# MasterXiong/Hyper-VLA

Measured on AMD Instinct MI355X. Metric: actions_per_sec, higher is better.
Workload: dtype f16; 1 GPU; BASELINE configs[1]: hypernet weight-gen once (untimed) + full sample_actions step (u8 224x224 -> DINOv2-base E=768 in the loop -> generated vit_t 4L/64d policy -> [4,7] action chunk); 1 action = 1 sample-step; batch_per_gpu=256, global_batch=256, encoder=DINOv2-base (reference parity, E=768), parallelism=episode-dp1 (no collectives), policy_operands=split-bf16 (bf16x3), launch=eager (114 launches per step, counted by the library), streams=1, ensemble=not in the step

## Files before the change

hyper-vla_amd/csrc/encoder.hip:

```cpp
#include <cstring>
#include <type_traits>

#include "common.h"
#include "kernels.h"
#include "plan.h"

namespace hvla {

template <typename Op>
__global__ void im2col_kernel(const uint8_t* __restrict__ img, typename Op::elem* __restrict__ out, int B,
                              int image, int patch, int grid, int Kp, float* __restrict__ x, const float* __restrict__ pos, int S, int E) {
  for (size_t i = (size_t)blockIdx.x * blockDim.x + threadIdx.x; i < (size_t)B * E; i += (size_t)gridDim.x * blockDim.x)
    x[(i / E) * S * E + (i % E)] = pos[i % E];
  const int Kp1 = Kp / 2, chunks = Kp1 / 8;
  const size_t total = (size_t)B * grid * grid * chunks;
  const int kreal = patch * patch * 3;
  for (size_t i = (size_t)blockIdx.x * blockDim.x + threadIdx.x; i < total; i += (size_t)gridDim.x * blockDim.x) {
    const int ch = (int)(i % chunks);
    const size_t m = i / chunks;
    const int px = (int)(m % grid), py = (int)((m / grid) % grid);
    const size_t b = m / ((size_t)grid * grid);
    typename Op::x8 v;
    const int rowb = 3 * patch;
    const int k0 = ch * 8;
    int dy = k0 / rowb, rb = k0 - dy * rowb;
    const uint8_t* src = img + ((b * image + (size_t)(py * patch + dy)) * image + (size_t)px * patch) * 3;
#pragma unroll
    for (int j = 0; j < 8; ++j) {
      float f = 0.f;
      if (k0 + j < kreal) f = (float)src[rb] - 128.f;
      v[j] = (typename Op::elem)f;
      if (++rb == rowb) rb = 0, src += (size_t)image * 3;
    }
    *reinterpret_cast<typename Op::x8*>(out + m * Kp + ch * 8) = v;
    *reinterpret_cast<typename Op::x8*>(out + m * Kp + Kp1 + ch * 8) = v;
  }
}

struct GemmArgs {
  const void* A;
  const void* W;
  int M, N, K;
  const float* bias;
  const float* aux;
  void* out;
  int P, S;
  int qcols;
  float qscale;
  const float* corr = nullptr;
  const void* abar2 = nullptr;
  const void* dW2 = nullptr;
  float* corr2 = nullptr;
  int M2 = 0;
  int row0 = 0, row_step = 1;
  int hsplit = 1 << 30;
  int tile_row0 = 0, tile_stride = 256, nbm = 0;
  void* colmean = nullptr;
  void* ln_out = nullptr;
  const float* ln_scale = nullptr;
  const float* ln_bias = nullptr;
  void* ln_abar = nullptr;
  uint32_t* ln_cnt = nullptr;
  float* ln_part = nullptr;
  uint32_t ln_target = 0;
  uint32_t ln_tag = 0;
  uint32_t ln_spin = 0;
  uint32_t out_bytes = 0;
  uint32_t part_bytes = 0;
  int lnx_G = 0, lnx_rows_aligned = 0, lnx_rounds_div = 0, lnx_rows_xcd = 0, lnx_rcp = 0;
  const float* ln_partial = nullptr;
};

__device__ __forceinline__ int wperm(int rho) { return (rho & ~63) + 4 * (rho & 15) + ((rho >> 4) & 3); }
__device__ __forceinline__ f32x4 corr_value(f32x4 acc, float b) {
  return f32x4{fmaf(acc[0], 1.f / 4096.f, b), fmaf(acc[1], 1.f / 4096.f, b), fmaf(acc[2], 1.f / 4096.f, b), fmaf(acc[3], 1.f / 4096.f, b)};
}

template <typename Op, int EPI, int MT, bool FULL, bool ROWBIAS, bool CS = false, bool WT = false, bool NT = false>
__device__ __forceinline__ void gemm_epilogue_rows_impl(const f32x4 (&acc)[4][MT], const GemmArgs& g, int m_base, int n_base,
                                                        int fr, int fq, const f32x4* pre_b4, const f32x4* pre_l4,
                                                        typename Op::x4* cs = nullptr,
                                                        const __attribute__((address_space(3))) float* lds_corr = nullptr,
                                                        int lds_img0 = -1) {
  using T = typename Op::elem;
  const int n = n_base + 4 * fr;
  f32x4 b4 = f32x4{0.f, 0.f, 0.f, 0.f};
  if constexpr (!ROWBIAS) b4 = pre_b4 ? *pre_b4 : *reinterpret_cast<const f32x4*>(g.bias + n);
  f32x4 l4 = f32x4{1.f, 1.f, 1.f, 1.f};
  if constexpr (EPI == EPI_RES) l4 = pre_l4 ? *pre_l4 : *reinterpret_cast<const f32x4*>(g.aux + n);
  const float q = EPI == EPI_PATCH ? g.qscale : ((EPI == EPI_QKV && n_base < g.qcols) ? g.qscale : 1.f);
  __amdgpu_buffer_rsrc_t wt_rsrc;
  if constexpr (WT) wt_rsrc = __builtin_amdgcn_make_buffer_rsrc(g.out, 0, (int)g.out_bytes, 0x00020000);
  auto store_f32x4 = [&](uint32_t elem_off, f32x4 v) {
    if constexpr (WT) __builtin_amdgcn_raw_buffer_store_b128(__builtin_bit_cast(u32x4, v), wt_rsrc, (int)(elem_off * 4u), 0, 16);
    else *reinterpret_cast<f32x4*>(reinterpret_cast<float*>(g.out) + elem_off) = v;
  };
  __amdgpu_buffer_rsrc_t nt_rsrc;
  uint32_t nt_vo = 0;
  if constexpr (NT && FULL && (EPI == EPI_QKV || EPI == EPI_GELU)) {
    nt_rsrc = __builtin_amdgcn_make_buffer_rsrc(g.out, 0, -1, 0x00020000);
    nt_vo = ((uint32_t)(g.row0 + (m_base + 4 * fq) * g.row_step) * (uint32_t)g.N + (uint32_t)n) * (uint32_t)sizeof(T);
  }
  constexpr int RB = MT < 2 ? 1 : (EPI == EPI_RES && MT >= 4 ? 4 : 2);
#pragma unroll
  for (int mp = 0; mp < MT; mp += RB) {
    f32x4 xin[RB][4], brow[RB][4];
    uint32_t off[RB][4];
    bool ok[RB][4];
#pragma unroll
    for (int u = 0; u < RB; ++u)
#pragma unroll
      for (int r = 0; r < 4; ++r) {
        const int m = m_base + (mp + u) * 16 + 4 * fq + r;
        ok[u][r] = FULL || m < g.M;
        const int grow = g.row0 + m * g.row_step;
        off[u][r] = (uint32_t)grow * (uint32_t)g.N + (uint32_t)n;
        if constexpr (EPI == EPI_PATCH) {
          const int prow = 1 + (m % g.P);
// ... 34 lines not shown
        if constexpr (EPI == EPI_GELU) {
          const f32x2 g0 = gelu_erf2(f32x2{t[c][0], t[c][1]}), g1 = gelu_erf2(f32x2{t[c][2], t[c][3]});
          t[c] = f32x4{g0[0], g0[1], g1[0], g1[1]};
        }
      }
#pragma unroll
      for (int r = 0; r < 4; ++r) {
        if (!ok[u][r]) continue;
        if constexpr (EPI == EPI_QKV || EPI == EPI_GELU) {
          typename Op::x4 o;
#pragma unroll
          for (int c = 0; c < 4; ++c) o[c] = (T)t[c][r];
          if constexpr (CS) *cs += o;
          if constexpr (NT && FULL) {
            int rowb = g.row_step * g.N * (int)sizeof(T);
            asm volatile("" : "+s"(rowb));
            __builtin_amdgcn_raw_buffer_store_b64(__builtin_bit_cast(u32x2, o), nt_rsrc, (int)nt_vo, ((mp + u) * 16 + r) * rowb, 2);
          } else if constexpr (NT) __builtin_nontemporal_store(o, reinterpret_cast<typename Op::x4*>(reinterpret_cast<T*>(g.out) + off[u][r]));
          else *reinterpret_cast<typename Op::x4*>(reinterpret_cast<T*>(g.out) + off[u][r]) = o;
        } else if constexpr (EPI == EPI_RES) {
          f32x4 x = xin[u][r];
#pragma unroll
          for (int c = 0; c < 4; ++c) x[c] = fmaf(t[c][r], l4[c], x[c]);
          store_f32x4(off[u][r], x);
        } else if constexpr (EPI == EPI_CORR) {
          *reinterpret_cast<f32x4*>(reinterpret_cast<float*>(g.out) + off[u][r]) = f32x4{t[0][r], t[1][r], t[2][r], t[3][r]};
        } else {
          f32x4 x = xin[u][r];
#pragma unroll
          for (int c = 0; c < 4; ++c) x[c] += t[c][r];
          store_f32x4(off[u][r], x);
        }
      }
    }
  }
}

template <typename Op, int EPI, int MT>
__device__ __forceinline__ void gemm_epilogue_rows(const f32x4 (&acc)[4][MT], const GemmArgs& g, int m_base, int n_base,
                                                   int fr, int fq) {
  const bool full = m_base + 16 * MT <= g.M;
  if constexpr (EPI == EPI_PATCH || EPI == EPI_CORR) {
    if (full) gemm_epilogue_rows_impl<Op, EPI, MT, true, false>(acc, g, m_base, n_base, fr, fq, nullptr, nullptr);
    else gemm_epilogue_rows_impl<Op, EPI, MT, false, false>(acc, g, m_base, n_base, fr, fq, nullptr, nullptr);
  } else {
    if (g.corr) {
      if (full) gemm_epilogue_rows_impl<Op, EPI, MT, true, true>(acc, g, m_base, n_base, fr, fq, nullptr, nullptr);
      else gemm_epilogue_rows_impl<Op, EPI, MT, false, true>(acc, g, m_base, n_base, fr, fq, nullptr, nullptr);
    } else {
      if (full) gemm_epilogue_rows_impl<Op, EPI, MT, true, false>(acc, g, m_base, n_base, fr, fq, nullptr, nullptr);
      else gemm_epilogue_rows_impl<Op, EPI, MT, false, false>(acc, g, m_base, n_base, fr, fq, nullptr, nullptr);
    }
  }
}


template <typename Op, int EPI>
__global__ __launch_bounds__(256, 2) void gemm_kernel(GemmArgs g) {
  using T = typename Op::elem;
  using X8 = typename Op::x8;
  extern __shared__ __attribute__((aligned(16))) char smem[];
  T* As = reinterpret_cast<T*>(smem);
  T* Ws = As + 2 * GBM * GLD;
  const int tid = threadIdx.x, wave = tid >> 6, lane = tid & 63;
  const int wm = wave >> 1, wn = wave & 1;
  const int nbm = (g.M + GBM - 1) / GBM, nbn = g.N / GBN;
  const int bid = xcd_run(blockIdx.x, nbm * nbn);
  const int bm = bid % nbm, bn = bid / nbm;
  const int m0 = bm * GBM, n0 = bn * GBN;
  const T* A = reinterpret_cast<const T*>(g.A);
  const T* W = reinterpret_cast<const T*>(g.W);

  const int lrow = tid >> 3, lch = tid & 7;
  const T* ap[4];
  const T* wp[4];
#pragma unroll
  for (int i = 0; i < 4; ++i) {
    int m = m0 + lrow + 32 * i;
    m = m < g.M ? m : g.M - 1;
    ap[i] = A + (size_t)(g.row0 + m * g.row_step) * g.K + lch * 8;
    wp[i] = W + (size_t)(n0 + wperm(lrow + 32 * i)) * g.K + lch * 8;
  }
  X8 ra[4], rw[4];
  auto gload = [&](int kt) {
#pragma unroll
    for (int i = 0; i < 4; ++i) {
      ra[i] = *reinterpret_cast<const X8*>(ap[i] + kt * GBK);
      rw[i] = *reinterpret_cast<const X8*>(wp[i] + kt * GBK);
    }
  };
  auto sstore = [&](int buf) {
#pragma unroll
    for (int i = 0; i < 4; ++i) {
      *reinterpret_cast<X8*>(As + (buf * GBM + lrow + 32 * i) * GLD + lch * 8) = ra[i];
      *reinterpret_cast<X8*>(Ws + (buf * GBN + lrow + 32 * i) * GLD + lch * 8) = rw[i];
    }
  };

  f32x4 acc[4][4];
#pragma unroll
  for (int i = 0; i < 4; ++i)
#pragma unroll
    for (int j = 0; j < 4; ++j) acc[i][j] = f32x4{0.f, 0.f, 0.f, 0.f};

  const int KT = g.K / GBK;
  gload(0);
  sstore(0);
  __syncthreads();
  const int fr = lane & 15, fq = lane >> 4;
  for (int kt = 0; kt < KT; ++kt) {
    const int buf = kt & 1;
    if (kt + 1 < KT) gload(kt + 1);
    const T* as = As + (buf * GBM + wm * 64 + fr) * GLD + fq * 8;
    const T* ws = Ws + (buf * GBN + wn * 64 + fr) * GLD + fq * 8;
#pragma unroll
    for (int kk = 0; kk < 2; ++kk) {
      X8 fa[4], fw[4];
#pragma unroll
      for (int t = 0; t < 4; ++t) {
        fa[t] = *reinterpret_cast<const X8*>(as + t * 16 * GLD + kk * 32);
        fw[t] = *reinterpret_cast<const X8*>(ws + t * 16 * GLD + kk * 32);
      }
#pragma unroll
      for (int nt = 0; nt < 4; ++nt)
#pragma unroll
        for (int mt = 0; mt < 4; ++mt) acc[nt][mt] = Op::mma16(fa[mt], fw[nt], acc[nt][mt]);
    }
    if (kt + 1 < KT) sstore(buf ^ 1);
    __syncthreads();
  }

  gemm_epilogue_rows<Op, EPI, 4>(acc, g, m0 + wm * 64, n0 + wn * 64, fr, fq);
}

template <typename Op, int EPI, int NS = SNS>
__device__ __forceinline__ void gemm64_body(const GemmArgs& g, int bm, int bn) {
  using T = typename Op::elem;
  using X8 = typename Op::x8;
  extern __shared__ __attribute__((aligned(16))) char smem[];
  const int tid = threadIdx.x, lane = tid & 63;
  const int wave = __builtin_amdgcn_readfirstlane(tid >> 6);
  const int m0 = bm * SBM, n0 = bn * SBN;
  const T* A = reinterpret_cast<const T*>(g.A);
  const T* W = reinterpret_cast<const T*>(g.W);
  const int sch = ((lane & 7) ^ (lane >> 3)) * 8;
  uint32_t aoff[2], woff[2];
#pragma unroll
  for (int j = 0; j < 2; ++j) {
    const int rl = 32 * j + 8 * wave + (lane >> 3);
    int m = m0 + rl;
    m = m < g.M ? m : g.M - 1;
    aoff[j] = (uint32_t)(g.row0 + m * g.row_step) * (uint32_t)g.K + sch;
    woff[j] = (uint32_t)(n0 + wperm(rl)) * (uint32_t)g.K + sch;
  }
  const int KT = g.K / 64;
  auto issue = [&](int kt) {
    char* base = smem + (kt % NS) * 16384 + wave * 1024;
#pragma unroll
    for (int j = 0; j < 2; ++j) {
      __builtin_amdgcn_global_load_lds((const __attribute__((address_space(1))) void*)(A + aoff[j] + kt * 64),
                                       (__attribute__((address_space(3))) void*)(base + j * 4096), 16, 0, 0);
      __builtin_amdgcn_global_load_lds((const __attribute__((address_space(1))) void*)(W + woff[j] + kt * 64),
                                       (__attribute__((address_space(3))) void*)(base + 8192 + j * 4096), 16, 0, 0);
    }
  };
  f32x4 acc[4][1];
#pragma unroll
  for (int i = 0; i < 4; ++i) acc[i][0] = f32x4{0.f, 0.f, 0.f, 0.f};
  const int fr = lane & 15, fq = lane >> 4;
  const int sw0 = (fq ^ (fr & 7)) << 4, sw1 = ((fq + 4) ^ (fr & 7)) << 4;
  const int a_off = (wave * 16 + fr) * 128, w_off = 8192 + fr * 128;
#pragma unroll
  for (int s = 0; s < NS - 1; ++s)
    if (s < KT) issue(s);
  for (int kt = 0; kt < KT; ++kt) {
    const int issued = kt + NS - 1 < KT ? kt + NS - 1 : KT;
    switch (issued - kt - 1) {
      case 0: asm volatile("s_waitcnt vmcnt(0)" ::: "memory"); break;
      case 1: asm volatile("s_waitcnt vmcnt(4)" ::: "memory"); break;
      case 2: asm volatile("s_waitcnt vmcnt(8)" ::: "memory"); break;
      case 3: asm volatile("s_waitcnt vmcnt(12)" ::: "memory"); break;
      default: asm volatile("s_waitcnt vmcnt(16)" ::: "memory"); break;
    }
    __builtin_amdgcn_sched_barrier(0);
    __builtin_amdgcn_s_barrier();
    asm volatile("" ::: "memory");
    __builtin_amdgcn_sched_barrier(0);
    const char* lb = smem + (kt % NS) * 16384;
    X8 fa[2], fw[4][2];
    fa[0] = *reinterpret_cast<const X8*>(lb + a_off + sw0);
    fa[1] = *reinterpret_cast<const X8*>(lb + a_off + sw1);
#pragma unroll
    for (int nt = 0; nt < 4; ++nt) {
      fw[nt][0] = *reinterpret_cast<const X8*>(lb + w_off + nt * 2048 + sw0);
      fw[nt][1] = *reinterpret_cast<const X8*>(lb + w_off + nt * 2048 + sw1);
    }
    __builtin_amdgcn_sched_barrier(0);
    if (kt + NS - 1 < KT) issue(kt + NS - 1);
    asm volatile("s_waitcnt lgkmcnt(0)" ::: "memory");
    __builtin_amdgcn_sched_barrier(0);
#pragma unroll
    for (int kk = 0; kk < 2; ++kk)
#pragma unroll
      for (int nt = 0; nt < 4; ++nt) acc[nt][0] = Op::mma16(fa[kk], fw[nt][kk], acc[nt][0]);
  }
  gemm_epilogue_rows<Op, EPI, 1>(acc, g, m0 + wave * 16, n0, fr, fq);
}

template <typename Op, int EPI, int NS = SNS>
__global__ __launch_bounds__(256) void gemm64_kernel(GemmArgs g) {
  const int nbm1 = (g.M + SBM - 1) / SBM, nbm2 = (g.M2 + SBM - 1) / SBM, rt_all = nbm1 + nbm2;
  const int t = xcd_run(blockIdx.x, gridDim.x);
  const int bn = t / rt_all, bm = t - bn * rt_all;
  if (bm < nbm1) {
    gemm64_body<Op, EPI, NS>(g, bm, bn);
  } else {
    GemmArgs c = g;
    c.A = g.abar2; c.W = g.dW2; c.out = g.corr2; c.M = g.M2; c.row0 = 0; c.row_step = 1; c.corr = nullptr;
    gemm64_body<Op, EPI_CORR, NS>(c, bm - nbm1, bn);
  }
}

__device__ __forceinline__ f32x4 ln_half_sum(const f32x4* p, int n4) { return (p[0] + p[n4]) + (p[2 * n4] + p[3 * n4]); }
template <typename Op, int EPI, bool FOLD = false>
__global__ __launch_bounds__(256) void gemm64c_kernel(GemmArgs g) {
  constexpr int SST = FOLD ? SSTF : SSTC, PCS = FOLD ? 6 : 7;
  using T = typename Op::elem;
  using X8 = typename Op::x8;
  extern __shared__ __attribute__((aligned(16))) char smem[];
  const int tid = threadIdx.x, lane = tid & 63;
  const int wave = __builtin_amdgcn_readfirstlane(tid >> 6);
  const int nbm = (g.M + SBM - 1) / SBM;
  const int tix = xcd_run(blockIdx.x, gridDim.x), bm = tix % nbm, bn = tix / nbm;
  const int m0 = bm * SBM, n0 = bn * SBN;
  const T* A = reinterpret_cast<const T*>(g.A);
  const T* W = reinterpret_cast<const T*>(g.W);
  const T* dW = reinterpret_cast<const T*>(g.dW2);
  const T* AB = reinterpret_cast<const T*>(g.abar2);
  const int img0 = (g.row0 + m0 * g.row_step) / g.S;
  const int sch = ((lane & 7) ^ (lane >> 3)) * 8;
  uint32_t aoff[2], woff[2], boff;
#pragma unroll
  for (int j = 0; j < 2; ++j) {
    const int rl = 32 * j + 8 * wave + (lane >> 3);
    int m = m0 + rl;
    m = m < g.M ? m : g.M - 1;
    aoff[j] = (uint32_t)(g.row0 + m * g.row_step) * (uint32_t)g.K + sch;
    woff[j] = (uint32_t)(n0 + wperm(rl)) * (uint32_t)g.K + sch;
  }
  {
    int mr = img0 * 2 + 8 * wave + (lane >> 3);
    mr = mr < g.M2 ? mr : g.M2 - 1;
    boff = (uint32_t)mr * (uint32_t)g.K + sch;
  }
  const int KT = g.K / 64;
  const uint32_t lds0 = (uint32_t)(uintptr_t)(__attribute__((address_space(3))) char*)smem;
  auto dma = [&](const T* sb, uint32_t elem_off, uint32_t dst) {
    const uint32_t vo = elem_off * (uint32_t)sizeof(T);
    uint32_t keep;
    asm volatile("s_mov_b32 %0, m0\n\ts_mov_b32 m0, %3\n\ts_nop 0\n\tglobal_load_lds_dwordx4 %1, %2\n\ts_mov_b32 m0, %0"
                 : "=&s"(keep) : "v"(vo), "s"(sb), "s"(dst));
  };
  auto issue_at = [&](int kt, int slot) {
    const uint32_t base = lds0 + (uint32_t)((slot % SNSC) * SST + wave * 1024);
#pragma unroll
    for (int j = 0; j < 2; ++j) {
      dma(A, aoff[j] + kt * 64, base + j * 4096);
      dma(W, woff[j] + kt * 64, base + 8192 + j * 4096);
      dma(dW, woff[j] + kt * 64, base + 16384 + j * 4096);
    }
    if constexpr (!FOLD) dma(AB, boff + kt * 64, base + 24576);
  };
  f32x4 acc[4][1], acc2 = f32x4{0.f, 0.f, 0.f, 0.f};
#pragma unroll
  for (int i = 0; i < 4; ++i) acc[i][0] = f32x4{0.f, 0.f, 0.f, 0.f};
  const int fr = lane & 15, fq = lane >> 4;
  const int sw0 = (fq ^ (fr & 7)) << 4, sw1 = ((fq + 4) ^ (fr & 7)) << 4;
  const int a_off = (wave * 16 + fr) * 128, w_off = 8192 + fr * 128;
  const int d_off = 16384 + (wave * 16 + fr) * 128, b_off = 24576 + fr * 128;
#pragma unroll
  for (int s = 0; s < SNSC - 1; ++s) issue_at(s < KT ? s : KT - 1, s);
  char* mtab = smem + SNSC * SST;
  if constexpr (FOLD) {
    int mlast = m0 + SBM - 1;
    mlast = mlast < g.M ? mlast : g.M - 1;
    const int nr = 2 * ((g.row0 + mlast * g.row_step) / g.S - img0 + 1);
    const int n4 = g.K / 4;
    for (int it = tid; it < nr * n4; it += 256) {
      const int r = it / n4, c4 = it - r * n4, bh = img0 * 2 + r;
      const f32x4 t = ln_half_sum(reinterpret_cast<const f32x4*>(g.ln_partial + (size_t)bh * 4 * g.K) + c4, n4);
      const float inv = 1.f / (float)(g.P / 2);
      typename Op::x4 o;
#pragma unroll
      for (int j = 0; j < 4; ++j) o[j] = (T)(t[j] * inv);
      const int k = 4 * c4;
      *reinterpret_cast<typename Op::x4*>(mtab + (k >> 6) * 2048 + r * 128 + ((((k & 63) >> 3) ^ (r & 7)) << 4) + (k & 7) * 2) = o;
    }
  }
  struct Frags {
    X8 fa[2], fw[4][2], fb[2], fd[2];
  };
  auto read_frags = [&](int t, Frags& f) {
    const char* lb = smem + (t % SNSC) * SST;
    f.fa[0] = *reinterpret_cast<const X8*>(lb + a_off + sw0);
    f.fa[1] = *reinterpret_cast<const X8*>(lb + a_off + sw1);
#pragma unroll
    for (int nt = 0; nt < 4; ++nt) {
      f.fw[nt][0] = *reinterpret_cast<const X8*>(lb + w_off + nt * 2048 + sw0);
      f.fw[nt][1] = *reinterpret_cast<const X8*>(lb + w_off + nt * 2048 + sw1);
// ... 338 lines not shown
  const int bh = blockIdx.x, n4 = E / 4;
  if ((int)threadIdx.x >= n4) return;
  const f32x4 t = ln_half_sum(reinterpret_cast<const f32x4*>(partial + (size_t)bh * 4 * E) + threadIdx.x, n4);
  const float inv = 1.f / (float)(P / 2);
  typename Op::x4 o;
#pragma unroll
  for (int j = 0; j < 4; ++j) o[j] = (typename Op::elem)(t[j] * inv);
  reinterpret_cast<typename Op::x4*>(abar + (size_t)bh * E)[threadIdx.x] = o;
}
constexpr int PRO_DMA = 12, PRO_DMA_KT0 = 8;
template <int EPI> struct EpiVmem { static constexpr int min_ops = (EPI == EPI_RES || EPI == EPI_PATCH) ? 64 : 32; };

#ifdef HVLA_BENCH_HOOKS
__device__ unsigned long long g_lnx_dbg[8][256];
#endif
constexpr int LNX_STAT = 98304, LNX_MR = LNX_STAT + 8192, LNX_CTRL = LNX_MR + 2048;
typedef __attribute__((address_space(3))) char lds_char;
template <typename Op, int EPI, bool PERSIST, bool LNX = false, bool NTOUT = false>
__global__ __launch_bounds__(512) void gemm256p_kernel(GemmArgs g) {
  static_assert(!NTOUT || EPI != EPI_PATCH, "NTOUT: non-temporal stores of the 16-bit outputs (QKV, GELU) / loads of the residual rows (RES)");
  using T = typename Op::elem;
  using X8 = typename Op::x8;
  static_assert(!LNX || EPI == EPI_RES || EPI == EPI_PATCH, "the fused LayerNorm follows a GEMM that writes the residual stream");
  extern __shared__ __attribute__((aligned(16))) char smem[];
  const int tid = threadIdx.x, lane = tid & 63;
  const int wave = __builtin_amdgcn_readfirstlane(tid >> 6);
  const int wm = wave >> 2, wn = wave & 3;
  const int nbm = g.nbm, nbn = (g.N + HBN_ - 1) / HBN_;
  const int ntiles = nbm * nbn;
  const int GN = nbn % 4 == 0 ? 4 : (nbn % 3 == 0 ? 3 : (nbn % 2 == 0 ? 2 : 1));
  auto tile_origin = [&](int v, int& tm, int& n0) {
    const int q = ntiles / 8, r = ntiles % 8, xcd = v % 8;
    const int bid = (xcd < r ? xcd * (q + 1) : r * (q + 1) + (xcd - r) * q) + v / 8;
    constexpr int CH = 8;
    const int per_chunk = CH * nbn;
    const int chunk = bid / per_chunk, rc = bid % per_chunk;
    const int rows = (nbm - chunk * CH) < CH ? (nbm - chunk * CH) : CH;
    const int sc = rc / (rows * GN), r2 = rc % (rows * GN);
    tm = chunk * CH + r2 / GN;
    n0 = (sc * GN + r2 % GN) * HBN_;
  };
  bool later = false;
  int rnd = 0;
  int pend_img = -1;
  uint32_t pend_mark = 0;
  auto tile_origin_x = [&](int& tm, int& n0, bool& lat) {
    typedef const __attribute__((address_space(4))) GemmArgs* karg_ptr;
    karg_ptr ga = (karg_ptr)__builtin_amdgcn_kernarg_segment_ptr();
    asm volatile("" : "+s"(ga));
    const int xcd = (int)blockIdx.x & 7, w = (int)blockIdx.x >> 3;
    const int G = ga->lnx_G, rcp = ga->lnx_rcp, wq = (w * rcp) >> 16, rq = (rnd * rcp) >> 16;
    int row, col;
    if (wq < G) {
      row = rnd * G + wq; col = w - wq * nbn; lat = false;
    } else {
      row = ga->lnx_rows_aligned + (w - G * nbn) * ga->lnx_rounds_div + rq; col = rnd - rq * nbn; lat = col != nbn - 1;
    }
    tm = xcd * ga->lnx_rows_xcd + row;
    n0 = col * HBN_;
    ++rnd;
  };
  int vb = blockIdx.x, tm, n0;
  if constexpr (LNX && PERSIST) tile_origin_x(tm, n0, later);
  else tile_origin(vb, tm, n0);
  int m0 = g.tile_row0 + tm * g.tile_stride;
  const T* A = reinterpret_cast<const T*>(g.A);
  const T* W = reinterpret_cast<const T*>(g.W);
  const int srow = wave * 8 + (lane >> 3);
  const int sch = ((lane & 7) ^ (lane >> 3)) * 8;
  const uint32_t lane_a = ((uint32_t)srow * (uint32_t)g.K + sch) * (uint32_t)sizeof(T);
  const uint32_t lane_w = ((uint32_t)(wperm(srow)) * (uint32_t)g.K + sch) * (uint32_t)sizeof(T);
  const uint32_t lds0 = (uint32_t)(uintptr_t)(__attribute__((address_space(3))) char*)smem;
  const T* abase = A + (size_t)m0 * g.K;
  const T* wbase = W + (size_t)n0 * g.K;
  int wn0 = n0;
  const int KT = g.K / 64;
  auto stage = [&](auto hc, int kt) {
    constexpr int h = decltype(hc)::value;
    const int buf = kt & 1;
#pragma unroll
    for (int u = 0; u < 2; ++u) {
      const int j = 2 * (h & 1) + u;
      const int jw = (h < 2 || wn0 + 64 * j < g.N) ? j : 0;
      const T* sb = (h < 2 ? abase : wbase) + ((size_t)jw * 64 * g.K + kt * 64);
      const uint32_t dst = lds0 + (uint32_t)(buf * 65536 + wave * 1024 + (h >> 1) * 32768 + j * 8192);
      const uint32_t vo = h < 2 ? lane_a : lane_w;
      uint32_t keep;
      asm volatile("s_mov_b32 %0, m0\n\ts_mov_b32 m0, %3\n\ts_nop 0\n\tglobal_load_lds_dwordx4 %1, %2\n\ts_mov_b32 m0, %0"
                   : "=&s"(keep) : "v"(vo), "s"(sb), "s"(dst));
    }
  };
  f32x4 acc[4][8];
  const int fr = lane & 15, fq = lane >> 4;
  const int sw0 = ((fq) ^ (fr & 7)) << 4, sw1 = ((fq + 4) ^ (fr & 7)) << 4;
  const int a_off = (wm * 128 + fr) * 128, w_off = 32768 + (wn * 64 + fr) * 128;
  X8 fa0[8], fa1[8], fw0[4], fw1[4];
  auto rd_a = [&](X8 (&f)[8], const char* lb, int ah) {
#pragma unroll
    for (int t = 0; t < 4; ++t) {
      f[2 * t] = *reinterpret_cast<const X8*>(lb + a_off + (4 * ah + t) * 2048 + sw0);
      f[2 * t + 1] = *reinterpret_cast<const X8*>(lb + a_off + (4 * ah + t) * 2048 + sw1);
    }
  };
  auto rd_w = [&](X8 (&f)[4], const char* lb, int wh) {
#pragma unroll
    for (int t = 0; t < 2; ++t) {
      f[2 * t] = *reinterpret_cast<const X8*>(lb + w_off + (2 * wh + t) * 2048 + sw0);
      f[2 * t + 1] = *reinterpret_cast<const X8*>(lb + w_off + (2 * wh + t) * 2048 + sw1);
    }
  };
  auto quad = [&](const X8 (&fa)[8], const X8 (&fw)[4], auto ahc, auto whc) {
    constexpr int ah = decltype(ahc)::value, wh = decltype(whc)::value;
#pragma unroll
    for (int kk = 0; kk < 2; ++kk)
#pragma unroll
      for (int mt = 0; mt < 4; ++mt)
#pragma unroll
        for (int nt = 0; nt < 2; ++nt)
          acc[2 * wh + nt][4 * ah + mt] = Op::mma16(fa[2 * mt + kk], fw[2 * nt + kk], acc[2 * wh + nt][4 * ah + mt]);
  };
  using H0 = std::integral_constant<int, 0>;
  using H1 = std::integral_constant<int, 1>;
  using H2 = std::integral_constant<int, 2>;
  using H3 = std::integral_constant<int, 3>;
#define HVLA_BAR() do { __builtin_amdgcn_sched_barrier(0); __builtin_amdgcn_s_barrier(); __builtin_amdgcn_sched_barrier(0); } while (0)
  stage(H0{}, 0); stage(H1{}, 0); stage(H2{}, 0); stage(H3{}, 0);
  if (KT > 1) {
    stage(H0{}, 1); stage(H1{}, 1);
    asm volatile("s_waitcnt vmcnt(4)" ::: "memory");
  } else {
    asm volatile("s_waitcnt vmcnt(0)" ::: "memory");
  }
  auto ktile = [&](int kt, auto s1c, auto s2c) {
    constexpr bool S1 = decltype(s1c)::value, S2 = decltype(s2c)::value;
    const char* lb = smem + (kt & 1) * 65536;
    rd_w(fw0, lb, 0);
    rd_a(fa0, lb, 0);
    if constexpr (S1) stage(H2{}, kt + 1);
    HVLA_BAR();
    asm volatile("s_waitcnt lgkmcnt(0)" ::: "memory");
    quad(fa0, fw0, H0{}, H0{});
    HVLA_BAR();
    rd_w(fw1, lb, 1);
    rd_a(fa1, lb, 1);
    if constexpr (S1) stage(H3{}, kt + 1);
    asm volatile("s_waitcnt lgkmcnt(0)" ::: "memory");
    HVLA_BAR();
    quad(fa0, fw1, H0{}, H1{});
    HVLA_BAR();
    if constexpr (S2) stage(H0{}, kt + 2);
    HVLA_BAR();
    quad(fa1, fw1, H1{}, H1{});
    HVLA_BAR();
    if constexpr (S2) stage(H1{}, kt + 2);
    if constexpr (S2) asm volatile("s_waitcnt vmcnt(4)" ::: "memory");
    else if constexpr (S1) asm volatile("s_waitcnt vmcnt(0)" ::: "memory");
    HVLA_BAR();
    quad(fa1, fw0, H1{}, H0{});
    HVLA_BAR();
  };
  using Yes = std::integral_constant<bool, true>;
  using No = std::integral_constant<bool, false>;
  while (true) {
#pragma unroll
    for (int i = 0; i < 4; ++i)
#pragma unroll
      for (int j = 0; j < 8; ++j) acc[i][j] = f32x4{0.f, 0.f, 0.f, 0.f};
// ... 969 lines not shown
  for (size_t i = (size_t)blockIdx.x * blockDim.x + threadIdx.x; i < n8; i += (size_t)gridDim.x * blockDim.x) {
    const x8 v = reinterpret_cast<const x8*>(p)[i];
#pragma unroll
    for (int j = 0; j < 8; ++j) {
      const float f = fabsf((float)v[j]);
      if (!(f <= 3.0e38f)) ++bad;
      else mx = fmaxf(mx, f);
    }
  }
#pragma unroll
  for (int o = 32; o >= 1; o >>= 1) {
    mx = fmaxf(mx, __shfl_xor(mx, o, 64));
    bad += __shfl_xor(bad, o, 64);
  }
  if ((threadIdx.x & 63) == 0) {
    atomicMax(slot, __float_as_uint(mx));
    if (bad) atomicAdd(slot + 1, bad);
  }
}

template <typename Op>
struct EncKernels {
  typedef void (*Gemm)(GemmArgs);
  typedef decltype(&attention_kernel<Op, false>) Attn;
  static const Gemm* gemm() {
    static const Gemm t[NUM_GEMM_KERNELS] = {
#define HVLA_X(id, ...) __VA_ARGS__,
        HVLA_GEMM_KERNELS(HVLA_X)
#undef HVLA_X
    };
    return t;
  }
  static const Attn* attn() {
    static const Attn t[NUM_ATTN_KERNELS] = {attention_kernel<Op, false>, attention_kernel<Op, false, 8>, attention_kernel<Op, true>};
    return t;
  }
  static auto ln_group() { return layernorm_group_kernel<Op>; }
  static hipError_t raise_lds_limit() {
    auto raise = [](auto kern) { return hipFuncSetAttribute(reinterpret_cast<const void*>(kern), hipFuncAttributeMaxDynamicSharedMemorySize, (int)LDS_LIMIT); };
    hipError_t e = raise(ln_group());
    for (int k = 0; k < NUM_GEMM_KERNELS && e == hipSuccess; ++k) e = raise(gemm()[k]);
    for (int k = 0; k < NUM_ATTN_KERNELS && e == hipSuccess; ++k) e = raise(attn()[k]);
    return e;
  }
};

namespace {
struct DeviceInfo {
  bool attr[2] = {false, false};
  int ncu = 0;
};
DeviceInfo g_dev[64];
}
template <typename Op>
static hipError_t device_setup(int& ncu) {
  constexpr int opi = std::is_same<Op, OpBF16>::value ? 1 : 0;
  int dev = 0;
  hipError_t e = hipGetDevice(&dev);
  if (e != hipSuccess) return e;
  if (dev < 0 || dev >= 64) return hipErrorInvalidDevice;
  DeviceInfo& di = g_dev[dev];
  if (!di.attr[opi]) {
    if ((e = EncKernels<Op>::raise_lds_limit()) != hipSuccess) return e;
    di.attr[opi] = true;
  }
  if (!di.ncu && (hipDeviceGetAttribute(&di.ncu, hipDeviceAttributeMultiprocessorCount, dev) != hipSuccess || di.ncu <= 0)) di.ncu = 256;
  ncu = di.ncu;
  return hipSuccess;
}
static dim3 grid_of(const Launch& l) { return dim3(l.grid, l.grid_y); }

#define HVLA_LAUNCH(...) do { ++pf.nlaunch; hipLaunchKernelGGL(__VA_ARGS__); } while (0)
template <typename Op>
static hipError_t run_encoder(const Geom& g, const EncWeights& w, const EncWorkspace& ws, const uint8_t* images,
                              float* tokens, int B, hipStream_t st, Profiler* prof, bool keep_cls, uint32_t* audit) {
  Profiler none;
  Profiler& pf = prof ? *prof : none;
  using T = typename Op::elem;
  using Kern = EncKernels<Op>;
  const int P = g.P(), S = g.S(), E = g.E, F = g.enc_mlp, H = g.enc_heads, M = B * S;
  const bool comp = w.layer[0].dqkv != nullptr && ws.corr && ws.abar;
  EncSizes z{B, P, S, E, F, H, g.patch, g.enc_layers, 0, sizeof(T), comp, ws.ln_cnt != nullptr && ws.ln_part != nullptr, ws.amap != nullptr};
  const CallPlan call = plan_call(z);
  if (!call.ok) return hipErrorInvalidValue;
  hipError_t e = device_setup<Op>(z.ncu);
  if (e != hipSuccess) return e;
  const int hsplit = 1 + P / 2;
  bool ln_fused = false;
  uint32_t ln_launch = 0;
  const float* ln_partial = nullptr;
  auto gemm = [&](int epi, GemmArgs a, const void* dW, int cat, const float* ln_s = nullptr, const float* ln_b = nullptr, void* colmean = nullptr) -> bool {
    const GemmPlan p = plan_gemm(z, epi, a.N, a.K, cat, ln_s != nullptr, ln_partial != nullptr);
    if (p.small) {
      GemmArgs c = a;
      if (p.aligned) {
        c.M = B; c.row0 = 0; c.row_step = S;
        if (comp) { c.abar2 = ws.abar; c.dW2 = dW; c.corr2 = ws.corr; c.M2 = 2 * B; }
      } else {
        c = GemmArgs{ws.abar, dW, 2 * B, a.N, a.K, a.bias, nullptr, ws.corr, P, S, 0, 1.f};
      }
      pf.begin(p.small.cat, st);
      HVLA_LAUNCH(Kern::gemm()[p.small.kernel], grid_of(p.small), dim3(p.small.block), p.small.lds, st, c);
      pf.end(p.small.cat, st);
    }
    if (p.aligned) {
      a.nbm = p.nbm; a.tile_row0 = p.tile_row0; a.tile_stride = p.tile_stride; a.colmean = colmean;
      if (epi != EPI_PATCH) a.corr = comp ? ws.corr : nullptr;
    } else if (p.fused_bias) {
      a.abar2 = ws.abar; a.dW2 = dW; a.M2 = 2 * B;
      if (p.fold) { a.ln_partial = ln_partial; ln_partial = nullptr; }
    } else if (p.small) {
      a.corr = ws.corr;
    }
    if (p.ln_fused) {
      a.hsplit = hsplit;
      a.ln_out = ws.h; a.ln_scale = ln_s; a.ln_bias = ln_b; a.ln_abar = comp ? ws.abar : nullptr; a.ln_cnt = ws.ln_cnt; a.ln_part = ws.ln_part;
      a.out_bytes = (uint32_t)((size_t)M * E * 4);
      a.part_bytes = (uint32_t)((size_t)B * p.nbn * 256 * 16);
      a.ln_tag = ++ln_launch;
      a.ln_target = ln_launch * (uint32_t)p.nbn;
      a.ln_spin = ws.ln_spin;
      a.lnx_G = p.lnx_G; a.lnx_rows_aligned = p.lnx_rows_aligned; a.lnx_rounds_div = p.lnx_rounds_div; a.lnx_rows_xcd = p.lnx_rows_xcd; a.lnx_rcp = p.lnx_rcp;
    }
    ln_fused = p.ln_fused;
    const int bracket = epi == EPI_PATCH ? -1 : p.main.cat;
    pf.begin(bracket, st);
    HVLA_LAUNCH(Kern::gemm()[p.main.kernel], grid_of(p.main), dim3(p.main.block), p.main.lds, st, a);
    pf.end(bracket, st);
    return p.aligned;
  };
  auto layer_gemm = [&](const void* A, const void* Wt, int N, int K, const float* bias, const float* aux, void* out, int qcols) {
    GemmArgs a{A, Wt, M, N, K, bias, aux, out, P, S, qcols, qcols ? 0.125f * 1.4426950408889634f : 1.f / 256.f};
    a.hsplit = hsplit;
    return a;
  };
  auto layernorm = [&](const float* sc, const float* bi, int Nnext, void* scratch, int scratch_cols) {
    const NormPlan n = plan_norm(z, Nnext, scratch_cols);
    float* partial = n.partial ? reinterpret_cast<float*>(scratch) : nullptr;
    pf.begin(n.group.cat, st);
    HVLA_LAUNCH(Kern::ln_group(), grid_of(n.group), dim3(n.group.block), n.group.lds, st, ws.x, reinterpret_cast<T*>(ws.h), sc, bi, partial, S, P, E);
    if (n.fold) ln_partial = partial;
    else if (n.mean) HVLA_LAUNCH((layernorm_mean_kernel<Op>), grid_of(n.mean), dim3(n.mean.block), 0, st, partial, reinterpret_cast<T*>(ws.abar), P, E);
    pf.end(n.group.cat, st);
  };
  auto audit_of = [&](const void* buf, size_t n, int site) {
    if (!audit) return;
    HVLA_LAUNCH((absmax_kernel<T>), dim3(1024), dim3(256), 0, st, reinterpret_cast<const T*>(buf), n / 8, audit + 2 * site);
  };
  if (call.cnt_bytes) {
    if ((e = hipMemsetAsync(ws.ln_cnt, 0, call.cnt_bytes, st)) != hipSuccess) return e;
    if ((e = hipMemsetAsync(ws.ln_part, 0, call.part_bytes, st)) != hipSuccess) return e;
    pf.nlaunch += 2;
  }
  pf.begin(call.im2col.cat, st);
  HVLA_LAUNCH(im2col_kernel<Op>, grid_of(call.im2col), dim3(call.im2col.block), 0, st, images, reinterpret_cast<T*>(ws.g), B,
              g.image_size, g.patch, g.grid(), call.Kp, ws.x, w.pos, S, E);
  gemm(EPI_PATCH, GemmArgs{ws.g, w.w_patch, B * P, E, call.Kp, w.b_patch, w.pos, ws.x, P, S, 0, 1.f / 256.f}, nullptr, call.im2col.cat,
       g.enc_layers > 0 ? w.layer[0].ln1_s : nullptr, g.enc_layers > 0 ? w.layer[0].ln1_b : nullptr);
  pf.end(call.im2col.cat, st);
#ifdef HVLA_BENCH_HOOKS
  int products = 0;
#define HVLA_STOP_HERE() do { if (ws.stop_after > 0 && ++products == ws.stop_after) return hipGetLastError(); } while (0)
#else
#define HVLA_STOP_HERE() do { } while (0)
#endif
  for (int l = 0; l < g.enc_layers; ++l) {
    const EncLayerW& L = w.layer[l];
// ... 101 lines not shown
```

hyper-vla_amd/csrc/plan.h:

```cpp
#pragma once
#include <stddef.h>
#include <stdint.h>

#ifdef __HIPCC__
#define HVLA_HD __host__ __device__ __forceinline__
#else
#define HVLA_HD inline
#endif

namespace hvla {

HVLA_HD int xcd_run(int bid, int nwg) {
  const int q = nwg / 8, r = nwg % 8, xcd = bid % 8;
  return (xcd < r ? xcd * (q + 1) : r * (q + 1) + (xcd - r) * q) + bid / 8;
}

HVLA_HD bool big_output(size_t rows, size_t cols, size_t elem_bytes) { return rows * cols * elem_bytes >= ((size_t)96 << 20); }

HVLA_HD bool nt16_addressable(size_t rows, size_t cols, size_t elem_bytes) { return rows * cols * elem_bytes < ((size_t)1 << 32); }

enum { EPI_PATCH = 0, EPI_QKV = 1, EPI_GELU = 2, EPI_RES = 3, EPI_CORR = 4 };
constexpr int GBM = 128, GBN = 128, GBK = 64, GLD = 72;
constexpr int SBM = 64, SBN = 64, SNS = 6, SST = 16384;
constexpr int SNSC = 5, SSTC = 28672;
// ... 91 lines not shown
    const int Wx = z.ncu / 8, R = p.nbm * p.nbn / z.ncu;
    p.lnx_G = Wx / p.nbn; p.lnx_rows_aligned = R * p.lnx_G; p.lnx_rounds_div = R / p.nbn; p.lnx_rows_xcd = p.nbm / 8;
    p.lnx_rcp = (65536 + p.nbn - 1) / p.nbn;
  }
}
inline GemmPlan plan_gemm(const EncSizes& z, int epi, int N, int K, int cat, bool ln_follows, bool ln_partial) {
  GemmPlan p;
  const int B = z.B, ncu = z.ncu, M = epi == EPI_PATCH ? B * z.P : z.M();
  const bool fits32 = (size_t)M * K < (1ull << 31) && (epi == EPI_PATCH || (size_t)N * K < (1ull << 31));
  p.main.block = 256;
  p.main.cat = cat;
  p.nbn = ceil_div(N, HBN_);
  p.aligned = N % SBN == 0 && N >= HBN_ && M > G64_MAXM && fits32 &&
              (epi == EPI_PATCH ? M % HBM_ == 0 : z.P == HBM_ && K >= 128 && K % 64 == 0);
  if (p.aligned) {
    p.main.block = 512;
    p.main.lds = P256_LDS;
    if (epi == EPI_PATCH) {
      p.nbm = M / HBM_; p.tile_row0 = 0; p.tile_stride = HBM_;
      if (z.P == HBM_ && can_fuse_ln(z) && ln_follows) { plan_lnx(z, p, G256LN_PATCH); return p; }
    } else {
      int nblocks = ceil_div(B, SBM) * (N / SBN);
      if (z.comp) nblocks += ceil_div(2 * B, SBM) * (N / SBN);
      const bool two_per_cu = nblocks > ncu;
      p.small = Launch{two_per_cu ? G64S4_QKV - EPI_QKV + epi : G64_PATCH + epi, (unsigned)nblocks, 1, 256, (size_t)(two_per_cu ? 4 : SNS) * SST, CAT_COMP};
      p.nbm = B; p.tile_row0 = 1; p.tile_stride = z.S;
      if (epi == EPI_RES && ln_follows && can_fuse_ln(z)) {
        plan_lnx(z, p, big_output(M, N, sizeof(float)) ? G256LNNT_RES : G256LN_RES);
        return p;
      }
      if (big_output(M, N, epi == EPI_RES ? sizeof(float) : z.elem) && (epi == EPI_RES || nt16_addressable(M, N, z.elem))) {
        const bool persist = (B * p.nbn) % ncu == 0;
        p.main.kernel = G256NT_QKV + 2 * (epi - EPI_QKV) + persist;
        p.main.grid = persist ? ncu : B * p.nbn;
        return p;
      }
    }
    const bool persist = (p.nbm * p.nbn) % ncu == 0;
    p.main.kernel = G256_PATCH + 2 * epi + persist;
    p.main.grid = persist ? ncu : p.nbm * p.nbn;
    return p;
  }
  if (epi != EPI_PATCH && small_fused(z, N, K)) {
    const int nb64 = ceil_div(M, SBM) * (N / SBN);
    p.fused_bias = true;
    if (epi != EPI_RES && ln_partial) {
      p.fold = true;
      p.main.kernel = G64CF_QKV - EPI_QKV + epi; p.main.grid = nb64; p.main.lds = gemm64c_fold_lds(K);
    } else if (epi == EPI_RES && 2 * nb64 <= ncu) {
      p.main.kernel = G64C32; p.main.grid = 2 * nb64; p.main.lds = (size_t)SNS32 * SST32;
    } else {
      p.main.kernel = G64C_QKV - EPI_QKV + epi; p.main.grid = nb64; p.main.lds = (size_t)SNSC * SSTC;
    }
    return p;
  }
  if (epi != EPI_PATCH && z.comp)
    p.small = Launch{G64_CORR, (unsigned)(ceil_div(2 * B, SBM) * (N / SBN)), 1, 256, (size_t)SNS * SST, CAT_COMP};
  if (M <= G64_MAXM && fits32 && N % SBN == 0 && (epi == EPI_PATCH || K % 64 == 0)) {
    p.main.kernel = G64_PATCH + epi; p.main.grid = ceil_div(M, SBM) * (N / SBN); p.main.lds = (size_t)SNS * SST;
  } else {
    p.main.kernel = G128_PATCH + epi; p.main.grid = ceil_div(M, GBM) * (N / GBN); p.main.lds = (size_t)2 * (GBM + GBN) * GLD * z.elem;
  }
  return p;
}

struct NormPlan {
  Launch group, mean;
  bool partial = false, fold = false;
};
inline NormPlan plan_norm(const EncSizes& z, int Nnext, int scratch_cols) {
  NormPlan n;
  n.group = Launch{LN_GROUP, LNG, (unsigned)z.B, LNW * 64, (size_t)(z.P / 8) * z.E * sizeof(float), 1};
  n.partial = z.comp && (size_t)LNG * z.E * sizeof(float) <= (size_t)z.S * scratch_cols * z.elem;
  n.fold = n.partial && small_fused(z, Nnext, z.E) && gemm64c_fold_lds(z.E) <= LDS_LIMIT && ceil_div(z.M(), SBM) * (Nnext / SBN) <= z.ncu;
  if (n.partial && !n.fold) n.mean = Launch{LN_MEAN, 2u * z.B, 1, 256, 0, 1};
  return n;
}

inline Launch plan_attention(int B, int S, int H, size_t elem, bool amap) {
  const int KT = (S + 31) / 32;
  return Launch{amap ? ATT_MAP : KT == 9 ? ATT_U : ATT, (unsigned)(B * H), 1, (unsigned)(KT - 1) * 64, attention_lds(KT, elem, amap), 3};
}

struct CallPlan {
  bool ok = false;
  int Kp = 0;
  size_t cnt_bytes = 0, part_bytes = 0;
  Launch im2col, attention, colmean, final_norm;
};
inline CallPlan plan_call(const EncSizes& z) {
  CallPlan c;
  const int M = z.M();
  c.ok = (size_t)M * (size_t)(z.F > 3 * z.E ? z.F : 3 * z.E) < (1ull << 32);
  if (!c.ok) return c;
  c.Kp = 2 * ((z.patch * z.patch * 3 + 63) / 64 * 64);
  if (can_fuse_ln(z) && z.P == HBM_ && M > G64_MAXM) {
    c.cnt_bytes = (size_t)((z.B * 4 + 15) / 16 * 16);
    c.part_bytes = (size_t)z.B * ceil_div(z.E, HBN_) * 256 * 16;
  }
  const size_t chunks = ((size_t)z.B * z.P * (c.Kp / 16) + 255) / 256;
  c.im2col = Launch{IM2COL, (unsigned)(chunks > 8192 ? 8192 : chunks), 1, 256, 0, 0};
  c.attention = plan_attention(z.B, z.S, z.H, z.elem, z.amap);
  if (z.comp) c.colmean = Launch{COLMEAN, (unsigned)ceil_div(z.F, 256), (unsigned)z.B, 256, 0, -1};
  c.final_norm = Launch{LN_FINAL, (unsigned)ceil_div(M, 4), 1, 256, 0, 1};
  return c;
}

}
```

Measured before the change: 19080 actions/s.

## Stage image strips in LDS for im2col and drop duplicated patch operand half

im2col now loads each full patch-row strip of the image into shared memory with aligned nontemporal 16-byte loads, then gathers patch elements from LDS instead of doing byte-wise global reads. It also writes only the first half of the split-bf16 patch operand. The patch GEMMs remap the A k-tile index for the second half back onto the first, so the duplicate copy is never materialised. This cuts global write traffic and uncoalesced reads in the patch-embedding stage, at the cost of a new LDS staging path with fallback conditions and a Kp%128 requirement.

Result: no change. 19110 actions/s, median of 6 (+0.2%).

```diff
diff --git a/hyper-vla_amd/csrc/encoder.hip b/hyper-vla_amd/csrc/encoder.hip
--- a/hyper-vla_amd/csrc/encoder.hip
+++ b/hyper-vla_amd/csrc/encoder.hip
@@ -7,21 +7,70 @@
 
 namespace hvla {
 
+constexpr int IM2COL_STRIP = 12288;
 template <typename Op>
 __global__ void im2col_kernel(const uint8_t* __restrict__ img, typename Op::elem* __restrict__ out, int B,
                               int image, int patch, int grid, int Kp, float* __restrict__ x, const float* __restrict__ pos, int S, int E) {
   for (size_t i = (size_t)blockIdx.x * blockDim.x + threadIdx.x; i < (size_t)B * E; i += (size_t)gridDim.x * blockDim.x)
     x[(i / E) * S * E + (i % E)] = pos[i % E];
   const int Kp1 = Kp / 2, chunks = Kp1 / 8;
+  const int kreal = patch * patch * 3;
+  const int rowb = 3 * patch, imgrow = 3 * image;
+  __shared__ __attribute__((aligned(16))) uint8_t strip[IM2COL_STRIP];
+  const int strip_bytes = patch * imgrow;
+  if (imgrow % 16 == 0 && (reinterpret_cast<uintptr_t>(img) & 15) == 0 && strip_bytes <= IM2COL_STRIP &&
+      strip_bytes <= 48 * (int)blockDim.x && chunks <= (int)blockDim.x && grid * patch <= image) {
+    const int tid = threadIdx.x, nthr = blockDim.x;
+    const int rpp = nthr / chunks;
+    const int pxo = tid / chunks, ch = tid - pxo * chunks;
+    int off[8];
+    uint32_t live = 0;
+    {
+      const int k0 = ch * 8;
+      int dy = k0 / rowb, rb = k0 - dy * rowb;
+#pragma unroll
+      for (int j = 0; j < 8; ++j) {
+        const bool real = k0 + j < kreal;
+        off[j] = real ? dy * imgrow + rb : 0;
+        live |= real ? 1u << j : 0u;
+        if (++rb == rowb) rb = 0, ++dy;
+      }
+    }
+    const int pieces = strip_bytes / 16;
+    for (int s = blockIdx.x; s < B * grid; s += gridDim.x) {
+      const int b = s / grid, py = s - b * grid;
+      const u32x4* src = reinterpret_cast<const u32x4*>(img + ((size_t)b * image + (size_t)py * patch) * imgrow);
+      u32x4 pc[3];
+#pragma unroll
+      for (int i = 0; i < 3; ++i)
+        if (tid + i * nthr < pieces) pc[i] = __builtin_nontemporal_load(src + tid + i * nthr);
+#pragma unroll
+      for (int i = 0; i < 3; ++i)
+        if (tid + i * nthr < pieces) reinterpret_cast<u32x4*>(strip)[tid + i * nthr] = pc[i];
+      __syncthreads();
+      if (pxo < rpp) {
+        for (int px = pxo; px < grid; px += rpp) {
+          const uint8_t* p = strip + px * rowb;
+          typename Op::x8 v;
+#pragma unroll
+          for (int j = 0; j < 8; ++j) {
+            const float f = (float)p[off[j]] - 128.f;
+            v[j] = (typename Op::elem)((live >> j) & 1u ? f : 0.f);
+          }
+          *reinterpret_cast<typename Op::x8*>(out + ((size_t)s * grid + px) * Kp + ch * 8) = v;
+        }
+      }
+      __syncthreads();
+    }
+    return;
+  }
   const size_t total = (size_t)B * grid * grid * chunks;
-  const int kreal = patch * patch * 3;
   for (size_t i = (size_t)blockIdx.x * blockDim.x + threadIdx.x; i < total; i += (size_t)gridDim.x * blockDim.x) {
     const int ch = (int)(i % chunks);
     const size_t m = i / chunks;
     const int px = (int)(m % grid), py = (int)((m / grid) % grid);
     const size_t b = m / ((size_t)grid * grid);
     typename Op::x8 v;
-    const int rowb = 3 * patch;
     const int k0 = ch * 8;
     int dy = k0 / rowb, rb = k0 - dy * rowb;
     const uint8_t* src = img + ((b * image + (size_t)(py * patch + dy)) * image + (size_t)px * patch) * 3;
@@ -33,7 +82,6 @@
       if (++rb == rowb) rb = 0, src += (size_t)image * 3;
     }
     *reinterpret_cast<typename Op::x8*>(out + m * Kp + ch * 8) = v;
-    *reinterpret_cast<typename Op::x8*>(out + m * Kp + Kp1 + ch * 8) = v;
   }
 }
 
@@ -234,10 +282,12 @@
     wp[i] = W + (size_t)(n0 + wperm(lrow + 32 * i)) * g.K + lch * 8;
   }
   X8 ra[4], rw[4];
+  const int KT = g.K / GBK;
   auto gload = [&](int kt) {
+    const int kta = EPI == EPI_PATCH ? patch_a_ktile(kt, KT) : kt;
 #pragma unroll
     for (int i = 0; i < 4; ++i) {
-      ra[i] = *reinterpret_cast<const X8*>(ap[i] + kt * GBK);
+      ra[i] = *reinterpret_cast<const X8*>(ap[i] + kta * GBK);
       rw[i] = *reinterpret_cast<const X8*>(wp[i] + kt * GBK);
     }
   };
@@ -255,7 +305,6 @@
 #pragma unroll
     for (int j = 0; j < 4; ++j) acc[i][j] = f32x4{0.f, 0.f, 0.f, 0.f};
 
-  const int KT = g.K / GBK;
   gload(0);
   sstore(0);
   __syncthreads();
@@ -308,9 +357,10 @@
   const int KT = g.K / 64;
   auto issue = [&](int kt) {
     char* base = smem + (kt % NS) * 16384 + wave * 1024;
+    const int kta = EPI == EPI_PATCH ? patch_a_ktile(kt, KT) : kt;
 #pragma unroll
     for (int j = 0; j < 2; ++j) {
-      __builtin_amdgcn_global_load_lds((const __attribute__((address_space(1))) void*)(A + aoff[j] + kt * 64),
+      __builtin_amdgcn_global_load_lds((const __attribute__((address_space(1))) void*)(A + aoff[j] + kta * 64),
                                        (__attribute__((address_space(3))) void*)(base + j * 4096), 16, 0, 0);
       __builtin_amdgcn_global_load_lds((const __attribute__((address_space(1))) void*)(W + woff[j] + kt * 64),
                                        (__attribute__((address_space(3))) void*)(base + 8192 + j * 4096), 16, 0, 0);
@@ -377,6 +427,7 @@
 template <typename Op, int EPI, bool FOLD = false>
 __global__ __launch_bounds__(256) void gemm64c_kernel(GemmArgs g) {
   constexpr int SST = FOLD ? SSTF : SSTC, PCS = FOLD ? 6 : 7;
+  static_assert(EPI != EPI_PATCH, "the patch product has no form with bias rows inside (it would need plan.h patch_a_ktile for its one operand copy)");
   using T = typename Op::elem;
   using X8 = typename Op::x8;
   extern __shared__ __attribute__((aligned(16))) char smem[];
@@ -881,7 +932,8 @@
     for (int u = 0; u < 2; ++u) {
       const int j = 2 * (h & 1) + u;
       const int jw = (h < 2 || wn0 + 64 * j < g.N) ? j : 0;
-      const T* sb = (h < 2 ? abase : wbase) + ((size_t)jw * 64 * g.K + kt * 64);
+      const int ktc = (EPI == EPI_PATCH && h < 2) ? patch_a_ktile(kt, KT) : kt;
+      const T* sb = (h < 2 ? abase : wbase) + ((size_t)jw * 64 * g.K + ktc * 64);
       const uint32_t dst = lds0 + (uint32_t)(buf * 65536 + wave * 1024 + (h >> 1) * 32768 + j * 8192);
       const uint32_t vo = h < 2 ? lane_a : lane_w;
       uint32_t keep;
@@ -2017,7 +2069,7 @@
   const bool comp = w.layer[0].dqkv != nullptr && ws.corr && ws.abar;
   EncSizes z{B, P, S, E, F, H, g.patch, g.enc_layers, 0, sizeof(T), comp, ws.ln_cnt != nullptr && ws.ln_part != nullptr, ws.amap != nullptr};
   const CallPlan call = plan_call(z);
-  if (!call.ok) return hipErrorInvalidValue;
+  if (!call.ok || call.Kp % 128) return hipErrorInvalidValue;
   hipError_t e = device_setup<Op>(z.ncu);
   if (e != hipSuccess) return e;
   const int hsplit = 1 + P / 2;
diff --git a/hyper-vla_amd/csrc/plan.h b/hyper-vla_amd/csrc/plan.h
--- a/hyper-vla_amd/csrc/plan.h
+++ b/hyper-vla_amd/csrc/plan.h
@@ -197,6 +197,9 @@
   return Launch{amap ? ATT_MAP : KT == 9 ? ATT_U : ATT, (unsigned)(B * H), 1, (unsigned)(KT - 1) * 64, attention_lds(KT, elem, amap), 3};
 }
 
+HVLA_HD int patch_kp(int patch) { return 2 * ((patch * patch * 3 + 63) / 64 * 64); }
+HVLA_HD int patch_a_ktile(int kt, int KT) { return kt < KT / 2 ? kt : kt - KT / 2; }
+
 struct CallPlan {
   bool ok = false;
   int Kp = 0;
@@ -208,7 +211,7 @@
   const int M = z.M();
   c.ok = (size_t)M * (size_t)(z.F > 3 * z.E ? z.F : 3 * z.E) < (1ull << 32);
   if (!c.ok) return c;
-  c.Kp = 2 * ((z.patch * z.patch * 3 + 63) / 64 * 64);
+  c.Kp = patch_kp(z.patch);
   if (can_fuse_ln(z) && z.P == HBM_ && M > G64_MAXM) {
     c.cnt_bytes = (size_t)((z.B * 4 + 15) / 16 * 16);
     c.part_bytes = (size_t)z.B * ceil_div(z.E, HBN_) * 256 * 16;
```
